# warlock-labs/sylow

Hardware: AMD Instinct MI355X
Metric: BN254 pairings/s (value) and BLS verifies/s (config.bls_verifies_per_s) at batch=2^20 per GPU (higher is better)
Workload: dtype i32/u32 limbs (9x29-bit carry-free core + 8x32-bit Montgomery, exact integer)

## Files before the change

sylow_amd/csrc/bn254_pair29.hpp:

```cpp
#pragma once
#include "bn254_f29.hpp"
#include "bn254_pair.hpp"

namespace bn254 {
namespace pl {

struct W2 { F29 c; };
BN_DEV const F29& f29_of(const W2& a) { return a.c; }
BN_DEV F29& f29_of(W2& a) { return a.c; }
struct W6 { W2 c0, c1, c2; };
struct W12 { W6 c0, c1; };

BN_DEV F29 xchg9(const F29& a) {
  F29 r;
#pragma unroll
  for (int i = 0; i < 9; ++i) r.v[i] = (i32)swap_u32((u32)a.v[i]);
  return r;
}
BN_DEV F29 sel9(bool odd, const F29& if_even, const F29& if_odd) {
  F29 r;
#pragma unroll
  for (int i = 0; i < 9; ++i) r.v[i] = odd ? if_odd.v[i] : if_even.v[i];
  return r;
}
BN_DEV F29 f29_reduce(const F29& a) {
  const F29* const x[1] = {&a};
  const i32 k[1] = {bn_keep(1)};
  return f29_reduce_terms(x, k);
}

#define BN_DPP_SWAP "row_half_mirror row_mask:0xf bank_mask:0xf"
#define BN_DPP_SWAP_C0 "row_half_mirror row_mask:0xf bank_mask:0x5"
#define BN_DPP_SELF_C0 "quad_perm:[0,1,2,3] row_mask:0xf bank_mask:0x5"
BN_DEV void w2_exchange(const F29& a, F29& b, F29& U, F29& W) {
  asm("s_nop 1\n\ts_mov_b32 vcc_lo, 0x0f0f0f0f\n\ts_mov_b32 vcc_hi, 0x0f0f0f0f\n\t"
      "v_cndmask_b32_dpp %0, %9, %9, vcc " BN_DPP_SWAP "\n\tv_cndmask_b32_dpp %1, %10, %10, vcc " BN_DPP_SWAP "\n\t"
      "v_cndmask_b32_dpp %2, %11, %11, vcc " BN_DPP_SWAP "\n\tv_cndmask_b32_dpp %3, %12, %12, vcc " BN_DPP_SWAP "\n\t"
      "v_cndmask_b32_dpp %4, %13, %13, vcc " BN_DPP_SWAP "\n\tv_cndmask_b32_dpp %5, %14, %14, vcc " BN_DPP_SWAP "\n\t"
      "v_cndmask_b32_dpp %6, %15, %15, vcc " BN_DPP_SWAP "\n\tv_cndmask_b32_dpp %7, %16, %16, vcc " BN_DPP_SWAP "\n\t"
// ... 14 lines not shown
      "v_mov_b32_dpp %0, %0 " BN_DPP_SWAP_C0 "\n\tv_mov_b32_dpp %1, %1 " BN_DPP_SWAP_C0 "\n\t"
      "v_mov_b32_dpp %2, %2 " BN_DPP_SWAP_C0 "\n\tv_mov_b32_dpp %3, %3 " BN_DPP_SWAP_C0 "\n\t"
      "v_mov_b32_dpp %4, %4 " BN_DPP_SWAP_C0 "\n\tv_mov_b32_dpp %5, %5 " BN_DPP_SWAP_C0 "\n\t"
      "v_mov_b32_dpp %6, %6 " BN_DPP_SWAP_C0 "\n\tv_mov_b32_dpp %7, %7 " BN_DPP_SWAP_C0 "\n\t"
      "v_mov_b32_dpp %8, %8 " BN_DPP_SWAP_C0 "\n\t"
      "v_sub_u32_dpp %0, %9, %0 " BN_DPP_SELF_C0 "\n\tv_sub_u32_dpp %1, %9, %1 " BN_DPP_SELF_C0 "\n\t"
      "v_sub_u32_dpp %2, %9, %2 " BN_DPP_SELF_C0 "\n\tv_sub_u32_dpp %3, %9, %3 " BN_DPP_SELF_C0 "\n\t"
      "v_sub_u32_dpp %4, %9, %4 " BN_DPP_SELF_C0 "\n\tv_sub_u32_dpp %5, %9, %5 " BN_DPP_SELF_C0 "\n\t"
      "v_sub_u32_dpp %6, %9, %6 " BN_DPP_SELF_C0 "\n\tv_sub_u32_dpp %7, %9, %7 " BN_DPP_SELF_C0 "\n\t"
      "v_sub_u32_dpp %8, %9, %8 " BN_DPP_SELF_C0
      : "+v"(b.v[0]), "+v"(b.v[1]), "+v"(b.v[2]), "+v"(b.v[3]), "+v"(b.v[4]), "+v"(b.v[5]), "+v"(b.v[6]), "+v"(b.v[7]), "+v"(b.v[8])
      : "v"(zero));
}
BN_NOINLINE F29 w2_mul_leaf(i32 a0, i32 a1, i32 a2, i32 a3, i32 a4, i32 a5, i32 a6, i32 a7, i32 a8,
                            i32 b0, i32 b1, i32 b2, i32 b3, i32 b4, i32 b5, i32 b6, i32 b7, i32 b8) {
  const F29 a{{a0, a1, a2, a3, a4, a5, a6, a7, a8}};
  F29 b{{b0, b1, b2, b3, b4, b5, b6, b7, b8}}, U, W;
  w2_exchange(a, b, U, W);
  return f29_dot2(a, U, W, b);
}
BN_NOINLINE F29 w2_mul_ilp_leaf(i32 a0, i32 a1, i32 a2, i32 a3, i32 a4, i32 a5, i32 a6, i32 a7, i32 a8,
                                i32 b0, i32 b1, i32 b2, i32 b3, i32 b4, i32 b5, i32 b6, i32 b7, i32 b8) {
  const F29 a{{a0, a1, a2, a3, a4, a5, a6, a7, a8}};
  F29 b{{b0, b1, b2, b3, b4, b5, b6, b7, b8}}, U, W;
  w2_exchange(a, b, U, W);
  return f29_dot2_ilp(a, U, W, b);
}
BN_NOINLINE F29 w2_sqr_leaf(i32 a0, i32 a1, i32 a2, i32 a3, i32 a4, i32 a5, i32 a6, i32 a7, i32 a8) {
  const F29 a{{a0, a1, a2, a3, a4, a5, a6, a7, a8}};
  const bool odd = lane_odd();
  const F29 o = xchg9(a);
  return f29_mul(sel9(odd, f29_add(a, o), o), sel9(odd, f29_sub(a, o), f29_dbl(a)));
}
BN_DEV W2 w2_mul(const W2& a, const W2& b) { return W2{w2_mul_leaf(W_ARGS(a.c), W_ARGS(b.c))}; }
BN_DEV W2 w2_mul_inl(const W2& a, const W2& bin) {
  F29 b = bin.c, U, W;
  w2_exchange(a.c, b, U, W);
  return W2{f29_dot2(a.c, U, W, b)};
}
BN_DEV W2 w2_mul_ilp(const W2& a, const W2& b) { return W2{w2_mul_ilp_leaf(W_ARGS(a.c), W_ARGS(b.c))}; }
BN_DEV W2 w2_sqr(const W2& a) { return W2{w2_sqr_leaf(W_ARGS(a.c))}; }
BN_DEV W2 w2_scale(const W2& a, const F29& k) { return W2{f29_mul_leaf(W_ARGS(a.c), W_ARGS(k))}; }

#ifndef BN_QUAD
#define BN_QUAD 0
#endif
#if BN_QUAD
template <class T> BN_DEV int quad_pair(T t) { return (int)((t & 3) ^ (((t >> 2) & 1) ? 3 : 0)); }
template <class T> BN_DEV T quad_index(T t) { return (T)(((t >> 3) << 1) | (T)(quad_pair(t) >> 1)); }
template <class T> BN_DEV int quad_sub(T t) { return quad_pair(t) & 1; }
BN_DEV bool quad_sub1() { return quad_sub(__lane_id()) != 0; }
BN_DEV F29 quad_xchg9(const F29& a) {
  F29 r;
#pragma unroll
  for (int i = 0; i < 9; ++i) r.v[i] = __builtin_amdgcn_mov_dpp(a.v[i], 0xB1, 0xF, 0xF, true);
  return r;
}
BN_DEV void quad_share(W2& r0, W2& r1, const F29& mine) {
  const bool s = quad_sub1();
  const F29 other = quad_xchg9(mine);
  r0 = W2{sel9(s, mine, other)};
  r1 = W2{sel9(s, other, mine)};
}
#endif
#if BN_QUAD
BN_DEV void w2_mul2(W2& r0, W2& r1, const W2& a0, const W2& b0, const W2& a1, const W2& b1) {
// ... 19 lines not shown
#define W2_SQR_MUL(r0, r1, a0, a1, b1) do { (r0) = w2_sqr(a0); (r1) = w2_mul(a1, b1); } while (0)
#define W2_SCALE2(r0, r1, a0, k0, a1, k1) do { (r0) = w2_scale(a0, k0); (r1) = w2_scale(a1, k1); } while (0)
#endif

BN_DEV W2 w2_add(const W2& a, const W2& b) { return W2{f29_add(a.c, b.c)}; }
BN_DEV W2 w2_sub(const W2& a, const W2& b) { return W2{f29_sub(a.c, b.c)}; }
BN_DEV W2 w2_neg(const W2& a) { return W2{f29_neg(a.c)}; }
BN_DEV W2 w2_norm(const W2& a) { return W2{f29_norm(a.c)}; }
BN_DEV W2 w2_reduce(const W2& a) { return W2{f29_reduce(a.c)}; }
BN_DEV W2 w2_lin2(const W2& a, int ka, const W2& b, int kb) { return W2{f29_lin2(a.c, ka, b.c, kb)}; }
BN_DEV W2 w2_xi_lin(const W2& x, int k, const W2& y, int m) {
  const F29 xo = xchg9(x.c);
  if (m == 0) {
    const F29* const t[2] = {&x.c, &xo};
    const i32 c[2] = {bn_keep(9 * k), bn_keep_v(lane_odd() ? k : -k)};
    return W2{f29_reduce_terms(t, c)};
  }
  const F29* const t[3] = {&x.c, &xo, &y.c};
  const i32 c[3] = {bn_keep(9 * k), bn_keep_v(lane_odd() ? k : -k), bn_keep(m)};
  return W2{f29_reduce_terms(t, c)};
}

BN_DEV W2 w2_from_s2(const S2& a) { return W2{f29_reduce(f29_from_fp(a.c))}; }
BN_DEV S2 w2_to_s2(const W2& a) { return S2{f29_to_fp(a.c)}; }
BN_DEV W2 w2_const(const uint32_t (&c)[2][8]) { return w2_from_s2(s2_const(c)); }
BN_DEV void w12_from_s12(W12& r, const S12& a) {
  r.c0.c0 = w2_from_s2(a.c0.c0); r.c0.c1 = w2_from_s2(a.c0.c1); r.c0.c2 = w2_from_s2(a.c0.c2);
  r.c1.c0 = w2_from_s2(a.c1.c0); r.c1.c1 = w2_from_s2(a.c1.c1); r.c1.c2 = w2_from_s2(a.c1.c2);
}
BN_DEV void w12_to_s12(S12& r, const W12& a) {
  r.c0.c0 = w2_to_s2(a.c0.c0); r.c0.c1 = w2_to_s2(a.c0.c1); r.c0.c2 = w2_to_s2(a.c0.c2);
  r.c1.c0 = w2_to_s2(a.c1.c0); r.c1.c1 = w2_to_s2(a.c1.c1); r.c1.c2 = w2_to_s2(a.c1.c2);
}

struct W6Raw { W2 v0, x0, y1, v2, y2; };
template <bool INL = false> BN_DEV W2 w2_mul_sel(const W2& a, const W2& b) { return INL ? w2_mul_inl(a, b) : w2_mul(a, b); }
template <bool INL = false>
BN_DEV W6Raw w6_mul_raw(const W6& a, const W6& b) {
  W2 v0, v1, v2, s0, s1, s2;
  W2_MUL2_SEL(INL, v0, v1, a.c0, b.c0, a.c1, b.c1);
  W2_MUL2_SEL(INL, v2, s0, a.c2, b.c2, w2_sub(a.c1, a.c2), w2_sub(b.c1, b.c2));
  W2_MUL2_SEL(INL, s1, s2, w2_sub(a.c0, a.c1), w2_sub(b.c0, b.c1), w2_sub(a.c0, a.c2), w2_sub(b.c0, b.c2));
  return W6Raw{v0, w2_sub(w2_add(v1, v2), s0), w2_sub(w2_add(v0, v1), s1), v2, w2_add(w2_sub(w2_add(v0, v2), s2), v1)};
}
template <bool INL = false>
BN_DEV W6 w6_mul(const W6& a, const W6& b) {
  const W6Raw m = w6_mul_raw<INL>(a, b);
  W6 r;
  r.c0 = w2_xi_lin(m.x0, 1, m.v0, 1);
  r.c1 = w2_xi_lin(m.v2, 1, m.y1, 1);
  r.c2 = w2_reduce(m.y2);
  return r;
}
BN_DEV W6 w6_add_norm(const W6& a, const W6& b) {
  return W6{w2_norm(w2_add(a.c0, b.c0)), w2_norm(w2_add(a.c1, b.c1)), w2_norm(w2_add(a.c2, b.c2))};
}
BN_DEV W6 w6_sub(const W6& a, const W6& b) { return W6{w2_sub(a.c0, b.c0), w2_sub(a.c1, b.c1), w2_sub(a.c2, b.c2)}; }

BN_DEV void w12_mul_c1(W12& r, const W6Raw& t2, const W6& t0, const W6& t1) {
  r.c1.c0 = w2_xi_lin(t2.x0, 1, w2_sub(w2_sub(t2.v0, t0.c0), t1.c0), 1);
  r.c1.c1 = w2_xi_lin(t2.v2, 1, w2_sub(w2_sub(t2.y1, t0.c1), t1.c1), 1);
  r.c1.c2 = w2_lin2(w2_sub(t2.y2, t0.c2), 1, t1.c2, -1);
}
BN_DEV W12 w12_mul(const W12& a, const W12& b) {
  const W6 t0 = w6_mul(a.c0, b.c0);
  const W6 t1 = w6_mul(a.c1, b.c1);
// ... 83 lines not shown
  W2 d0, d2, d4, p12, p54, p10, p34, p30, p52, q02, q24, q04;
  W2_MUL2(d0, d2, z0, x0, z2, x2);
  W2_MUL2(d4, p12, z4, x4, z1, x2);
  W2_MUL2(p54, p10, z5, x4, z1, x0);
  W2_MUL2(p34, p30, z3, x4, z3, x0);
  W2_MUL2(p52, q02, z5, x2, w2_sub(z0, z2), w2_sub(x0, x2));
  W2_MUL2(q24, q04, w2_sub(z2, z4), w2_sub(x2, x4), w2_sub(z0, z4), w2_sub(x0, x4));
  const W2 qs = w2_mul(w2_norm(w2_add(w2_add(z1, z3), z5)), w2_norm(w2_add(w2_add(x0, x2), x4)));
  W12 o;
  o.c0.c0 = w2_xi_lin(w2_add(p12, d4), 1, d0, 1);
  o.c0.c1 = w2_xi_lin(w2_add(p54, d2), 1, p10, 1);
  o.c0.c2 = w2_reduce(w2_add(w2_sub(w2_add(d0, d2), q02), p34));
  o.c1.c0 = w2_xi_lin(w2_sub(w2_add(d2, d4), q24), 1, p30, 1);
  o.c1.c1 = w2_xi_lin(p52, 1, w2_sub(w2_add(d0, d4), q04), 1);
  {
    const W2 sa = w2_add(w2_add(p12, p54), p10), sb = w2_add(w2_add(p34, p30), p52);
    const F29* const t[3] = {&qs.c, &sa.c, &sb.c};
    const i32 c[3] = {bn_keep(1), bn_keep(-1), bn_keep(-1)};
    o.c1.c2 = W2{f29_reduce_terms(t, c)};
  }
  return o;
}
BN_DEV W2 w2_xi_lin_v(const W2& x, const W2& y, i32 m) {
  const F29 xo = xchg9(x.c);
  const F29* const t[3] = {&x.c, &xo, &y.c};
  const i32 c[3] = {bn_keep(9), bn_keep_v(lane_odd() ? 1 : -1), bn_keep_v(m)};
  return W2{f29_reduce_terms(t, c)};
}
BN_DEV W2 w2_lin_v(const W2& x, const W2& y, i32 m) {
  const F29* const t[2] = {&x.c, &y.c};
  const i32 c[2] = {bn_keep(1), bn_keep_v(m)};
  return W2{f29_reduce_terms(t, c)};
}
BN_DEV W12 w12_sparse_mul_unit(const W12& f, i32 u, const W2& x4, const W2& x2) {
  const W2 z0 = f.c0.c0, z1 = f.c0.c1, z2 = f.c0.c2, z3 = f.c1.c0, z4 = f.c1.c1, z5 = f.c1.c2;
  W2 d2, d4, p12, p54, p34, p52, a02, a04, q24, q13;
  W2_MUL2(d2, d4, z2, x2, z4, x4);
  W2_MUL2(p12, p54, z1, x2, z5, x4);
  W2_MUL2(p34, p52, z3, x4, z5, x2);
  W2_MUL2(a02, a04, z0, x2, z0, x4);
  const W2 x24 = w2_sub(x2, x4);
  W2_MUL2(q24, q13, w2_sub(z2, z4), x24, w2_sub(z1, z3), x24);
  W12 o;
  o.c0.c0 = w2_xi_lin_v(w2_add(p12, d4), z0, u);
  o.c0.c1 = w2_xi_lin_v(w2_add(p54, d2), z1, u);
  o.c0.c2 = w2_lin_v(w2_add(a02, p34), z2, u);
  o.c1.c0 = w2_xi_lin_v(w2_sub(w2_add(d2, d4), q24), z3, u);
  {
    const F29 xo = xchg9(p52.c);
    const F29* const t[4] = {&p52.c, &xo, &a04.c, &z4.c};
    const i32 c[4] = {bn_keep(9), bn_keep_v(lane_odd() ? 1 : -1), bn_keep(1), bn_keep_v(u)};
    o.c1.c1 = W2{f29_reduce_terms(t, c)};
  }
  o.c1.c2 = w2_lin_v(w2_sub(w2_add(p12, p34), q13), z5, u);
  return o;
}
BN_DEV W2 w2_xi_norm(const W2& x, const W2& y) {
  const F29 xo = xchg9(x.c);
  const F29* const t[3] = {&x.c, &xo, &y.c};
  const i32 c[3] = {bn_keep(9), bn_keep_v(lane_odd() ? 1 : -1), bn_keep(1)};
  return W2{f29_norm_terms(t, c)};
}
BN_DEV W2 w2_xi_norm_sub(const W2& x, const W2& y) {
  const F29 xo = xchg9(x.c);
  const F29* const t[3] = {&x.c, &xo, &y.c};
  const i32 c[3] = {bn_keep(-9), bn_keep_v(lane_odd() ? -1 : 1), bn_keep(1)};
  return W2{f29_norm_terms(t, c)};
}
template <bool INL = false>
BN_DEV void w_fp4_square_fold(W2& out0, W2& m, const W2& a, const W2& b, const W2& z) {
  W2 w;
  W2_MUL2_SEL(INL, m, w, a, b, w2_sub(a, b), w2_xi_norm_sub(b, a));
  const F29 mo = xchg9(m.c);
  const F29* const t[4] = {&w.c, &m.c, &mo, &z.c};
  const i32 c[4] = {bn_keep(3), bn_keep(30), bn_keep_v(lane_odd() ? 3 : -3), bn_keep(-2)};
  out0 = W2{f29_reduce_terms(t, c)};
}
template <bool INL = false>
BN_DEV W12 w12_cyclotomic_sqr(const W12& f) {
  const W2 z0 = f.c0.c0, z4 = f.c0.c1, z3 = f.c0.c2, z2 = f.c1.c0, z1 = f.c1.c1, z5 = f.c1.c2;
  W2 m;
  W12 r;
  w_fp4_square_fold<INL>(r.c0.c0, m, z0, z1, z0);
  r.c1.c1 = w2_lin2(m, 6, z1, 2);
  w_fp4_square_fold<INL>(r.c0.c1, m, z2, z3, z4);
  r.c1.c2 = w2_lin2(m, 6, z5, 2);
  w_fp4_square_fold<INL>(r.c0.c2, m, z4, z5, z3);
  r.c1.c0 = w2_xi_lin(m, 6, z2, 2);
  return r;
}

BN_DEV F29 f29_halve(const F29& a) {
  i32 p[9]; f29_p(p);
  const i32 m = -(a.v[0] & 1);
  i32 lo[9];
  i32 c = 0;
#pragma unroll
  for (int i = 0; i < 8; ++i) {
    i32 t = a.v[i] + (p[i] & m) + c;
// ... 29 lines not shown
  W2 xy, xx, b, c, yz2, e;
  W2_MUL_SQR(xy, xx, r.x, r.y, r.x);
  const W2 a = w2_halve(xy);
  l2 = w2_norm(w2_triple(xx));
  W2_SQR2(b, c, r.y, r.z);
  if (ISO) {
    yz2 = w2_sqr(w2_norm(w2_add(r.y, r.z)));
    e = w2_mul_27m3u(c);
  } else {
    W2_SQR_MUL(yz2, e, w2_norm(w2_add(r.y, r.z)), w2_twist_b(), w2_norm(w2_triple(c)));
  }
  const W2 h = w2_norm(w2_sub(yz2, w2_add(b, c)));
  l1 = w2_neg(h);
  l0 = w2_xi_lin(w2_sub(e, b), 1, b, 0);
  const W2 f = w2_norm(w2_triple(e));
  W2_MUL2(r.z, r.x, b, h, a, w2_sub(b, f));
  const W2 g = w2_halve(w2_norm(w2_add(b, f)));
  W2 gg, ee;
  W2_SQR2(gg, ee, g, e);
  r.y = w2_lin2(gg, 1, ee, -3);
#else
  const W2 a = w2_halve(w2_mul(r.x, r.y));
  l2 = w2_norm(w2_triple(w2_sqr(r.x)));
  const W2 b = w2_sqr(r.y);
  const W2 c = w2_sqr(r.z);
  const W2 h = w2_norm(w2_sub(w2_sqr(w2_norm(w2_add(r.y, r.z))), w2_add(b, c)));
  const W2 e = ISO ? w2_mul_27m3u(c) : w2_mul(w2_twist_b(), w2_norm(w2_triple(c)));
  l1 = w2_neg(h);
  r.z = w2_mul(b, h);
  l0 = w2_xi_lin(w2_sub(e, b), 1, b, 0);
  const W2 f = w2_norm(w2_triple(e));
  r.x = w2_mul(a, w2_sub(b, f));
  const W2 g = w2_halve(w2_norm(w2_add(b, f)));
  r.y = w2_lin2(w2_sqr(g), 1, w2_sqr(e), -3);
#endif
}
BN_DEV void g2_addition_step29(G2W& r, const W2& bx, const W2& by, W2& l0, W2& l1, W2& l2) {
#if BN_QUAD
  W2 zbx, zby, ebx, dby;
  W2_MUL2(zbx, zby, r.z, bx, r.z, by);
  const W2 d = w2_sub(r.x, zbx);
  const W2 e = w2_sub(r.y, zby);
  W2_MUL2(ebx, dby, e, bx, d, by);
  l0 = w2_xi_lin(w2_sub(ebx, dby), 1, bx, 0);
  l1 = d;
  l2 = w2_neg(e);
  const W2 dn = w2_norm(d), en = w2_norm(e);
  W2 f, ee, h, i, zee, zh, dj, hy;
  W2_SQR2(f, ee, dn, en);
  W2_MUL2(h, i, dn, f, r.x, f);
  W2_MUL2(zee, zh, r.z, ee, r.z, h);
  const W2 j = w2_norm(w2_sub(w2_add(zee, h), w2_add(i, i)));
  W2_MUL2(dj, hy, dn, j, h, r.y);
  r.z = zh;
  r.x = dj;
  r.y = w2_norm(w2_sub(w2_mul(en, w2_sub(i, j)), hy));
#else
  const W2 d = w2_sub(r.x, w2_mul(r.z, bx));
  const W2 e = w2_sub(r.y, w2_mul(r.z, by));
  l0 = w2_xi_lin(w2_sub(w2_mul(e, bx), w2_mul(d, by)), 1, bx, 0);
  l1 = d;
  l2 = w2_neg(e);
  const W2 dn = w2_norm(d), en = w2_norm(e);
  const W2 f = w2_sqr(dn);
  const W2 h = w2_mul(dn, f);
  const W2 i = w2_mul(r.x, f);
  const W2 j = w2_norm(w2_sub(w2_add(w2_mul(r.z, w2_sqr(en)), h), w2_add(i, i)));
  r.z = w2_mul(r.z, h);
  r.x = w2_mul(dn, j);
  r.y = w2_norm(w2_sub(w2_mul(en, w2_sub(i, j)), w2_mul(h, r.y)));
#endif
}
BN_DEV W12 w12_line_product(const W2& a0, const W2& a4, const W2& a2, const W2& b0, const W2& b4, const W2& b2) {
  W2 d0, d2, d4, k02, k24, k04;
  W2_MUL2(d0, d2, a0, b0, a2, b2);
  W2_MUL2(d4, k02, a4, b4, w2_sub(a0, a2), w2_sub(b0, b2));
  W2_MUL2(k24, k04, w2_sub(a2, a4), w2_sub(b2, b4), w2_sub(a0, a4), w2_sub(b0, b4));
  W12 r;
  r.c0.c0 = w2_xi_lin(d4, 1, d0, 1);
  r.c0.c1 = w2_xi_lin(d2, 1, d2, 0);
  r.c0.c2 = w2_reduce(w2_sub(w2_add(d0, d2), k02));
  r.c1.c0 = w2_xi_lin(w2_sub(w2_add(d2, d4), k24), 1, d2, 0);
  r.c1.c1 = w2_reduce(w2_sub(w2_add(d0, d4), k04));
  r.c1.c2 = W2{F29{{0, 0, 0, 0, 0, 0, 0, 0, 0}}};
  return r;
}
constexpr int MILLER_LDS_WORDS = 36, MILLER_LDS_WORDS_PARK = 63;
BN_DEV void lds_put9(i32 (*lds)[256], int slot, const F29& a) {
#pragma unroll
  for (int i = 0; i < 9; ++i) lds[9 * slot + i][threadIdx.x] = a.v[i];
}
BN_DEV F29 lds_get9(i32 (*lds)[256], int slot) {
  F29 r;
#pragma unroll
  for (int i = 0; i < 9; ++i) r.v[i] = lds[9 * slot + i][threadIdx.x];
  return r;
}
#ifndef BN_MILLER_SQR_INL
#define BN_MILLER_SQR_INL false
#endif
template <bool PARK, bool ISO = false>
BN_NOINLINE void miller_loop29g(S12& fout, const Fp& pxs, const Fp& pys, const S2& qxs_in, const S2& qys_in) {
  __shared__ i32 lds[PARK ? MILLER_LDS_WORDS_PARK : MILLER_LDS_WORDS][256];
  S2 qxs = qxs_in, qys = qys_in;
  {
    const F29 px = f29_reduce(f29_from_fp(pxs)), py = f29_reduce(f29_from_fp(pys));
    lds_put9(lds, 0, ISO ? f29_mul(px, f29_iso_s2()) : px);
    lds_put9(lds, 1, ISO ? f29_mul(py, f29_iso_s3()) : py);
  }
  {
    W2 qx = w2_from_s2(qxs), qy = w2_from_s2(qys);
    if (ISO) {
      W2_SCALE2(qx, qy, qx, f29_iso_s2(), qy, f29_iso_s3());
      qxs = w2_to_s2(qx); qys = w2_to_s2(qy);
    }
    lds_put9(lds, 2, qx.c);
    lds_put9(lds, 3, qy.c);
  }
  auto PX = [&]() { return lds_get9(lds, 0); };
  auto PY = [&]() { return lds_get9(lds, 1); };
  auto QX = [&]() { return W2{lds_get9(lds, 2)}; };
  auto QY = [&](bool neg) { const W2 y{lds_get9(lds, 3)}; return neg ? w2_neg(y) : y; };
  auto park = [&](const G2W& r) { if (PARK) { lds_put9(lds, 4, r.x.c); lds_put9(lds, 5, r.y.c); lds_put9(lds, 6, r.z.c); } };
  auto unpark = [&](const G2W& r) { return PARK ? G2W{W2{lds_get9(lds, 4)}, W2{lds_get9(lds, 5)}, W2{lds_get9(lds, 6)}} : r; };
  W12 f;
  G2W r{QX(), QY(false), w2_from_s2(s2_one())};
  W2 l0, l1, l2;
  auto line_mul = [&](const W12& x) {
    W2 s1, s2;
    W2_SCALE2(s1, s2, l1, PY(), l2, PX());
    return w12_sparse_mul(x, l0, s1, s2);
  };
  const u64 nz = BN_ATE_NAF_NZ, ng = BN_ATE_NAF_NEG;
  static_assert((BN_ATE_NAF_NZ >> 63) & 1, "the first digit of 6x+2 after the leading one is non-zero");
  {
    g2_doubling_step29<ISO>(r, l0, l1, l2);
    const W2 d0 = l0;
    W2 d4, d2, e4, e2;
    W2_SCALE2(d4, d2, l1, PY(), l2, PX());
    g2_addition_step29(r, QX(), QY((ng >> 63) & 1), l0, l1, l2);
    park(r);
    W2_SCALE2(e4, e2, l1, PY(), l2, PX());
    f = w12_line_product(d0, d4, d2, l0, e4, e2);
  }
#pragma unroll 1
  for (int i = 1; i < 64; ++i) {
    r = unpark(r);
    g2_doubling_step29<ISO>(r, l0, l1, l2);
    park(r);
    f = w12_sqr<BN_MILLER_SQR_INL>(f);
    f = line_mul(f);
    if ((nz >> (63 - i)) & 1) {
      r = unpark(r);
      g2_addition_step29(r, QX(), QY((ng >> (63 - i)) & 1), l0, l1, l2);
      park(r);
      f = line_mul(f);
    }
  }
  r = unpark(r);
  S2 q1x, q1y, q2x, q2y;
  g2_psi_affine(q1x, q1y, qxs, qys);
  g2_psi_affine(q2x, q2y, q1x, q1y);
  q2y = s2_neg(q2y);
  g2_addition_step29(r, w2_from_s2(q1x), w2_from_s2(q1y), l0, l1, l2);
  f = line_mul(f);
  g2_addition_step29(r, w2_from_s2(q2x), w2_from_s2(q2y), l0, l1, l2);
  f = line_mul(f);
  w12_to_s12(fout, f);
}


BN_DEV void w12_pin(W12& x) {
  W2* const c[6] = {&x.c0.c0, &x.c0.c1, &x.c0.c2, &x.c1.c0, &x.c1.c1, &x.c1.c2};
#pragma unroll
  for (int j = 0; j < 6; ++j)
#pragma unroll
    for (int i = 0; i < 9; ++i) BN_CHAIN_NV(c[j]->c.v[i]);
}
BN_NOINLINE void w12_mul_nl(W12& r, const W12& a, const W12& b) {
  W12 x = a, y = b;
  w12_pin(x); w12_pin(y);
  r = w12_mul(x, y);
}
BN_NOINLINE void w12_cyclotomic_sqr_nl(W12& r, const W12& a) {
  W12 x = a;
  w12_pin(x);
  r = w12_cyclotomic_sqr(x);
}
template <int E> BN_NOINLINE void w12_frobenius_nl(W12& r, const W12& a) {
  W12 x = a;
  w12_pin(x);
  r = w12_frobenius<E>(x);
}
#ifndef BN_EXP_INL
#define BN_EXP_INL true
#endif
#define BN_X_C_NZ 0x0008144402208421ull
#define BN_X_C_NEG 0x0008004400000020ull
#define BN_X_C_17 0x0000100000008021ull
BN_NOINLINE void exp_by_neg_z29(W12& r, const W12& f) {
  W12 tab[2];
// ... 22 lines not shown
}
BN_DEV W2 w2_inv(const W2& a) {
  const F29 t = f29_mul_leaf(W_ARGS(a.c), W_ARGS(a.c));
  const F29 n = f29_norm(f29_add(t, xchg9(t)));
  const F29 i = f29_reduce(f29_from_fp(fp_inv(f29_to_fp(n))));
  const F29 r = f29_mul_leaf(W_ARGS(a.c), W_ARGS(i));
  return W2{sel9(lane_odd(), r, f29_norm(f29_neg(r)))};
}
BN_DEV W2 w2_mul_xi(const W2& a) { return w2_xi_lin(a, 1, a, 0); }
BN_DEV W6 w6_inv(const W6& a) {
  W2 s0, m12, s2, m01, s1, m02, u1, u2, o0, o1;
  W2_SQR_MUL(s0, m12, a.c0, a.c1, w2_mul_xi(a.c2));
  W2_SQR_MUL(s2, m01, a.c2, a.c0, a.c1);
  W2_SQR_MUL(s1, m02, a.c1, a.c0, a.c2);
  const W2 t0 = w2_sub(s0, m12);
  const W2 t1 = w2_sub(w2_mul_xi(s2), m01);
  const W2 t2 = w2_sub(s1, m02);
  W2_MUL2(u1, u2, a.c2, t1, a.c1, t2);
  const W2 d = w2_xi_lin(w2_add(u1, u2), 1, w2_mul(a.c0, t0), 1);
  const W2 di = w2_inv(d);
  W2_MUL2(o0, o1, di, t0, di, t1);
  return W6{o0, o1, w2_mul(di, t2)};
}
BN_NOINLINE void w12_inv_nl(W12& r, const W12& ain) {
  W12 a = ain;
  w12_pin(a);
  const W6 s0 = w6_mul(a.c0, a.c0), s1 = w6_mul(a.c1, a.c1);
  const W6 d{w2_norm(w2_sub(s0.c0, w2_mul_xi(s1.c2))), w2_norm(w2_sub(s0.c1, s1.c0)), w2_norm(w2_sub(s0.c2, s1.c1))};
  const W6 t = w6_inv(d);
  r.c0 = w6_mul(a.c0, t);
  const W6 m = w6_mul(a.c1, t);
  r.c1 = W6{w2_norm(w2_neg(m.c0)), w2_norm(w2_neg(m.c1)), w2_norm(w2_neg(m.c2))};
}
BN_NOINLINE void final_exponentiation29(S12& out, const S12& fin) {
  W12 in, t, a, b, d, e, g;
  {
    w12_from_s12(t, fin);
    w12_inv_nl(b, t);
    a = w12_conj(t);
    w12_mul_nl(d, a, b);
    w12_frobenius_nl<2>(a, d);
    w12_mul_nl(in, a, d);
  }
  exp_by_neg_z29(a, in);
  w12_cyclotomic_sqr_nl(b, a);
  w12_cyclotomic_sqr_nl(t, b);
  w12_mul_nl(d, t, b);
  exp_by_neg_z29(e, d);
  w12_cyclotomic_sqr_nl(t, e);
  exp_by_neg_z29(g, t);
  d = w12_conj(d);
  g = w12_conj(g);
  w12_mul_nl(t, g, e);
  w12_mul_nl(a, t, d);
  w12_mul_nl(d, a, b);
  w12_mul_nl(t, a, e);
  w12_mul_nl(e, in, t);
  w12_frobenius_nl<1>(t, d);
  w12_mul_nl(b, t, e);
  w12_frobenius_nl<2>(t, a);
  w12_mul_nl(e, t, b);
  t = w12_conj(in);
  w12_mul_nl(a, t, d);
  w12_frobenius_nl<3>(t, a);
  w12_mul_nl(g, t, e);
  w12_to_s12(out, g);
}


#ifdef BN_WIDE_LEAF_CALL
BN_DEV W2 w2_mul_w(const W2& a, const W2& b) { return w2_mul(a, b); }
#else
BN_DEV W2 w2_mul_w(const W2& a, const W2& b) { return w2_mul_inl(a, b); }
#endif
struct alignas(16) WideLds { i32 v[63][2][12]; };
typedef __attribute__((address_space(3))) WideLds* WideLdsPtr;
template <int EPW> BN_DEV int wide_j(int lane) { return (int)pair_index((u32)lane) & (32 / EPW - 1); }
typedef i32 __attribute__((ext_vector_type(4))) WideVec4;
typedef __attribute__((address_space(3))) WideVec4* WideVec4Ptr;
BN_DEV void wide_put(WideLdsPtr x, int slot, int odd, const W2& a) {
  const WideVec4Ptr p = (WideVec4Ptr)&x->v[slot][odd][0];
  p[0] = WideVec4{a.c.v[0], a.c.v[1], a.c.v[2], a.c.v[3]};
  p[1] = WideVec4{a.c.v[4], a.c.v[5], a.c.v[6], a.c.v[7]};
  x->v[slot][odd][8] = a.c.v[8];
}
BN_DEV W2 wide_get(WideLdsPtr x, int slot, int odd) {
  const WideVec4Ptr p = (WideVec4Ptr)&x->v[slot][odd][0];
  const WideVec4 lo = p[0], hi = p[1];
  W2 r;
  r.c.v[0] = lo.x; r.c.v[1] = lo.y; r.c.v[2] = lo.z; r.c.v[3] = lo.w;
  r.c.v[4] = hi.x; r.c.v[5] = hi.y; r.c.v[6] = hi.z; r.c.v[7] = hi.w;
  r.c.v[8] = x->v[slot][odd][8];
  return r;
}
BN_DEV W2 w2_pick(const W2& a, const W2& b, bool c) { return W2{sel9(c, a.c, b.c)}; }
BN_DEV W2 w2_real(const F29& k) { return W2{sel9(lane_odd(), k, F29{{0, 0, 0, 0, 0, 0, 0, 0, 0}})}; }
BN_DEV W2 w2_sel3(int k, const W2& a, const W2& b, const W2& c) { return w2_pick(w2_pick(a, b, k == 1), c, k == 2); }
template <int EPW = 1>
BN_DEV W12 w12_cyclotomic_sqr_wide(const W12& f, WideLdsPtr x) {
// ... 427 lines not shown
```

sylow_amd/csrc/plk_pairing.hip:

```cpp
#include "plk_common.hpp"

namespace plk {
__global__ void HEAVY_BOUNDS k_miller_loop(const u64* pxy, const u64* qxy, u64* fout, size_t n) {
  const size_t t = TID, i = pair_index(t);
  const int odd = pair_role(t);
  if (i >= n) return;
  const Fp px = load_fp(pxy, n, i, 0), py = load_fp(pxy, n, i, 4);
  const S2 qx = load_s2(qxy, n, i, 0, odd), qy = load_s2(qxy, n, i, 8, odd);
  S12 f;
  miller_loop29g<true>(f, px, py, qx, qy);
  store_s12(fout, n, i, odd, f);
}
__global__ void HEAVY_BOUNDS k_final_exp(const u64* fin, u64* gout, size_t n) {
  const size_t t = TID, i = pair_index(t);
  const int odd = pair_role(t);
  if (i >= n) return;
  S12 f, g;
  load_s12(f, fin, n, i, odd);
  final_exponentiation29(g, f);
  store_s12(gout, n, i, odd, g);
}
BN_DEV void pairing_body(const u64* pxy, const uint8_t* pinf, const u64* qxy, const uint8_t* qinf, u64* gout, size_t n, size_t m, const Stagger& st) {
  unsigned chunk;
  int role = stagger_role(st, chunk);
  const size_t t = (size_t)chunk * blockDim.x + threadIdx.x, i = pair_index(t);
  const int odd = pair_role(t);
  const size_t np = (size_t)st.count * (BLOCK / 2), ip = (size_t)(chunk - st.first) * (BLOCK / 2) + (i & (BLOCK / 2 - 1));
  if (role == 2 && !stagger_wait(st, chunk)) role = 0;
  if (role == 2) {
    S12 f, g;
    load_s12(f, st.park, np, ip, odd);
    final_exponentiation29(g, f);
    store_s12(gout, n, i, odd, g);
    return;
  }
  if (i >= m) return;
  const bool either_zero = (pinf && pinf[i]) || (qinf && qinf[i]);
  S12 g;
  if (either_zero) {
    g = s12_one();
    if (role == 1) store_s12(st.park, np, ip, odd, g);
  } else {
    const Fp px = load_fp(pxy, n, i, 0), py = load_fp(pxy, n, i, 4);
    const S2 qx = load_s2(qxy, n, i, 0, odd), qy = load_s2(qxy, n, i, 8, odd);
    S12 f;
    miller_loop29g<true, true>(f, px, py, qx, qy);
    if (role == 1) store_s12(st.park, np, ip, odd, f);
    else final_exponentiation29(g, f);
  }
  if (role == 1) { stagger_publish(st, chunk); return; }
  store_s12(gout, n, i, odd, g);
}
__global__ void HEAVY_BOUNDS k_pairing(const u64* pxy, const uint8_t* pinf, const u64* qxy, const uint8_t* qinf, u64* gout, size_t n, size_t m, Stagger st) {
  ClockProbe pb;
  probe_begin(pb, st.clk);
  pairing_body(pxy, pinf, qxy, qinf, gout, n, m, st);
  probe_end(pb, st.clk);
}

using namespace plkh;
__global__ void HEAVY_BOUNDS k_w12_op(int op, const u64* a, const u64* b, u64* out, size_t n) {
  const size_t t = TID, i = pair_index(t);
  const int odd = pair_role(t);
  if (i >= n) return;
  S12 sx, sy, sr;
  load_s12(sx, a, n, i, odd);
  if (op >= OPW_S_MUL && op <= OPW_S_CYCSQR) {
    if (b) load_s12(sy, b, n, i, odd);
    if (op == OPW_S_MUL) sr = s12_mul(sx, sy);
    else if (op == OPW_S_SQR) sr = s12_sqr(sx);
    else if (op == OPW_S_INV) sr = s12_inv(sx);
    else sr = cyclotomic_sqr(sx);
  } else {
    w12_hook_op(op - OPW_MUL, sr, sx, b, n, i, odd);
  }
  store_s12(out, n, i, odd, sr);
}
}

namespace plkh {
int32_t fp12_op(int32_t op, const uint64_t* a, const uint64_t* b, uint64_t* out, size_t n, void* stream) {
// ... 61 lines not shown
```

sylow_amd/csrc/plk_quad.hip:

```cpp
#define BN_QUAD 1
#include "plk_common.hpp"
#include "plk_verify_body.hpp"

namespace plk {
__global__ void HEAVY_BOUNDS k_pairing_quad(const u64* pxy, const uint8_t* pinf, const u64* qxy, const uint8_t* qinf, u64* gout, size_t n, size_t m, u64* clk) {
  const size_t t = TID, i = quad_index(t);
  const int odd = pair_role(t);
  if (i >= m) return;
  ClockProbe pb;
  probe_begin(pb, clk);
  __builtin_amdgcn_s_setprio(2);
  const bool either_zero = (pinf && pinf[i]) || (qinf && qinf[i]);
  S12 g;
  if (either_zero) {
    g = s12_one();
  } else {
    const Fp px = load_fp(pxy, n, i, 0), py = load_fp(pxy, n, i, 4);
    const S2 qx = load_s2(qxy, n, i, 0, odd), qy = load_s2(qxy, n, i, 8, odd);
    S12 f;
    miller_loop29g<true, true>(f, px, py, qx, qy);
    final_exponentiation29(g, f);
  }
  if (quad_sub(t) == 0) store_s12(gout, n, i, odd, g);
  probe_end(pb, clk);
}
__global__ void HEAVY_BOUNDS k_miller_loop_quad(const u64* pxy, const u64* qxy, u64* fout, size_t n) {
  const size_t t = TID, i = quad_index(t);
  const int odd = pair_role(t);
  if (i >= n) return;
  const Fp px = load_fp(pxy, n, i, 0), py = load_fp(pxy, n, i, 4);
  const S2 qx = load_s2(qxy, n, i, 0, odd), qy = load_s2(qxy, n, i, 8, odd);
  S12 f;
  miller_loop29g<true>(f, px, py, qx, qy);
  if (quad_sub(t) == 0) store_s12(fout, n, i, odd, f);
}
__global__ void HEAVY_BOUNDS k_final_exp_quad(const u64* fin, u64* gout, size_t n) {
  const size_t t = TID, i = quad_index(t);
  const int odd = pair_role(t);
  if (i >= n) return;
  S12 f, g;
  load_s12(f, fin, n, i, odd);
  final_exponentiation29(g, f);
  if (quad_sub(t) == 0) store_s12(gout, n, i, odd, g);
}
template <bool PK_TABLE>
__global__ void HEAVY_BOUNDS k_bls_verify_fused_quad(const u64* pkxy, const uint8_t* pkinf, const i32* pk_table, const u64* hneg, const uint8_t* hneg_inf,
                                                     const u64* sigxy, const uint8_t* siginf, const i32* gen_table, uint8_t* okout, size_t n, size_t m, u64* clk) {
  const Stagger none{0, 0, 0, 0, nullptr, nullptr, nullptr};
  __builtin_amdgcn_s_setprio(2);
  ClockProbe pb;
  probe_begin(pb, clk);
  bls_verify_fused_body<PK_TABLE>(pkxy, pkinf, pk_table, hneg, hneg_inf, sigxy, siginf, gen_table, okout, n, m, none);
// ... 48 lines not shown
```

sylow_amd/csrc/plk_verify.hip:

```cpp
#include "plk_common.hpp"
#include "plk_verify_body.hpp"

namespace plk {
BN_DEV bool hash_to_g1_pair(Fp& hx, Fp& hy, bool& hinf, const uint8_t* msg, size_t msg_len, const DstPrime& dp) {
  const bool odd = lane_odd();
  u64 em[12], half[6];
  expand_message_xmd96_words(em, msg, msg_len, dp);
#pragma unroll
  for (int k = 0; k < 6; ++k) half[k] = odd ? em[6 + k] : em[k];
  const Fp u = fp_from_be48_words(half);
  Fp x, y;
  u32 ok = svdw_map(x, y, u) ? 1u : 0u;
  ok &= swap_u32(ok);
  const Fp ox = xchg(x), oy = xchg(y);
  const G1P a{sel(odd, x, ox), sel(odd, y, oy), fp_one()}, b{sel(odd, ox, x), sel(odd, oy, y), fp_one()};
  const G1P h = g1_add(a, b);
  g1_to_affine(hx, hy, hinf, h);
  return ok != 0;
}

constexpr int LINES_BLOCK = 192;
__global__ void __launch_bounds__(LINES_BLOCK) k_g2_lines29(const u64* qxy, size_t n, size_t idx, i32* table) {
  __shared__ i32 raw[LINE_TABLE_LINES][3][2][9];
  const int odd = pair_role(threadIdx.x);
  if (pair_index(threadIdx.x) == 0) {
    S2 qxs = s2_g2gen_x(), qys = s2_g2gen_y();
    if (qxy) { qxs = load_s2(qxy, n, idx, 0, odd); qys = load_s2(qxy, n, idx, 8, odd); }
    const W2 qx = w2_from_s2(qxs), qy = w2_from_s2(qys), nqy = w2_from_s2(s2_neg(qys));
    G2W r{qx, qy, w2_from_s2(s2_one())};
    W2 l0, l1, l2;
    int at = 0;
    auto put = [&]() {
      const W2 c[3] = {l0, w2_reduce(l1), w2_reduce(l2)};
      for (int k = 0; k < 3; ++k) for (int j = 0; j < 9; ++j) raw[at][k][odd][j] = c[k].c.v[j];
      ++at;
    };
    const u64 nz = BN_ATE_NAF_NZ, ng = BN_ATE_NAF_NEG;
#pragma unroll 1
    for (int i = 0; i < 64; ++i) {
      g2_doubling_step29(r, l0, l1, l2); put();
      if ((nz >> (63 - i)) & 1) { g2_addition_step29(r, qx, ((ng >> (63 - i)) & 1) ? nqy : qy, l0, l1, l2); put(); }
    }
    S2 q1x, q1y, q2x, q2y;
    g2_psi_affine(q1x, q1y, qxs, qys);
    g2_psi_affine(q2x, q2y, q1x, q1y);
    g2_addition_step29(r, w2_from_s2(q1x), w2_from_s2(q1y), l0, l1, l2); put();
    g2_addition_step29(r, w2_from_s2(q2x), w2_from_s2(s2_neg(q2y)), l0, l1, l2); put();
  }
  __syncthreads();
  const int line = (int)(pair_index(threadIdx.x));
  if (line >= LINE_TABLE_LINES) return;
  auto get = [&](int k) {
    const i32* t = raw[line][k][odd];
    return W2{F29{{t[0], t[1], t[2], t[3], t[4], t[5], t[6], t[7], t[8]}}};
  };
  const W2 l0 = get(0), l1 = get(1), l2 = get(2);
  u32 nzero = 0;
  for (int j = 0; j < 9; ++j) nzero |= (u32)l0.c.v[j];
  nzero |= swap_u32(nzero);
  const bool unit = nzero != 0;
  const W2 inv = w2_inv(l0);
  const W2 c[2] = {unit ? w2_reduce(w2_mul(l1, inv)) : l1, unit ? w2_reduce(w2_mul(l2, inv)) : l2};
  for (int k = 0; k < 2; ++k) for (int j = 0; j < 9; ++j) table[((line * 2 + k) * 2 + odd) * 9 + j] = c[k].c.v[j];
  if (!odd) table[LINE_TABLE_LINES * 36 + line] = unit ? 1 : 0;
}
__global__ void HEAVY_BOUNDS k_bls_verify(const u64* pkxy, const uint8_t* pkinf, const uint8_t* msgs, const u64* off, DstPrime dp,
                                          const u64* sigxy, const uint8_t* siginf, const i32* gen_table, uint8_t* okout, size_t n) {
  __shared__ i32 tabA[LINE_TABLE_WORDS];
  stage_table(tabA, gen_table);
  __syncthreads();
  const size_t t = TID, i = pair_index(t);
  const int odd = pair_role(t);
  if (i >= n) return;
  Fp hx, hy; bool hinf;
  hash_to_g1_pair(hx, hy, hinf, msgs + off[i], (size_t)(off[i + 1] - off[i]), dp);
  S12 lhs, rhs;
  if (siginf && siginf[i]) {
    lhs = s12_one();
  } else {
    const F29 sx = f29_reduce(f29_from_fp(load_fp(sigxy, n, i, 0))), sy = f29_reduce(f29_from_fp(load_fp(sigxy, n, i, 4)));
// ... 222 lines not shown
```

sylow_amd/csrc/plk_verify_body.hpp:

```cpp
#pragma once
#include "plk_common.hpp"

namespace plk {
BN_DEV void stage_table(i32* lds, const i32* src) {
  for (int k = threadIdx.x; k < LINE_TABLE_WORDS; k += blockDim.x) lds[k] = src[k];
}
BN_DEV W2 table_w2(const i32* tab, int at, int c, int odd) {
  const i32* t = tab + ((at * 2 + c) * 2 + odd) * 9;
  return W2{F29{{t[0], t[1], t[2], t[3], t[4], t[5], t[6], t[7], t[8]}}};
}
BN_DEV i32 table_unit(const i32* tab, int at) { return tab[LINE_TABLE_LINES * 36 + at]; }

template <bool PK_TABLE>
BN_DEV void bls_verify_fused_body(const u64* pkxy, const uint8_t* pkinf, const i32* pk_table,
                                  const u64* hneg, const uint8_t* hneg_inf,
                                  const u64* sigxy, const uint8_t* siginf, const i32* gen_table, uint8_t* okout, size_t n, size_t m, const Stagger& st) {
  __shared__ i32 tabA[LINE_TABLE_WORDS];
  __shared__ i32 tabB[PK_TABLE ? LINE_TABLE_WORDS : 1];
  unsigned chunk;
  int role = stagger_role(st, chunk);
  const size_t t = (size_t)chunk * blockDim.x + threadIdx.x, i = elem_index(t);
  const int odd = pair_role(t);
  const size_t np = (size_t)st.count * ELEMS_PER_BLOCK, ip = (size_t)(chunk - st.first) * ELEMS_PER_BLOCK + (i & (ELEMS_PER_BLOCK - 1));
  if (role == 2 && !stagger_wait(st, chunk)) role = 0;
  if (role == 2) {
    S12 fs, g;
    load_s12(fs, st.park, np, ip, odd);
    final_exponentiation29(g, fs);
    const bool one = s12_is_one(g);
    if (!odd && elem_writer(t)) okout[i] = one ? 1 : 0;
    return;
  }
  stage_table(tabA, gen_table);
  if (PK_TABLE) stage_table(tabB, pk_table);
  __syncthreads();
  const bool active = i < m;
  const size_t ii = active ? i : 0;
  const Fp hxs = load_fp(hneg, n, ii, 0), hys = load_fp(hneg, n, ii, 4);
  const bool hinf = hneg_inf[ii] != 0;
  __shared__ i32 lds[PK_TABLE ? 36 : 54][256];
  const bool liveA = !(siginf && siginf[ii]);
  const bool liveB = !(hinf || (pkinf && pkinf[PK_TABLE ? 0 : ii]));
  const F29 f29_zero{{0, 0, 0, 0, 0, 0, 0, 0, 0}};
  lds_put9(lds, 0, liveA ? f29_reduce(f29_from_fp(load_fp(sigxy, n, ii, 0))) : f29_zero);
  lds_put9(lds, 1, liveA ? f29_reduce(f29_from_fp(load_fp(sigxy, n, ii, 4))) : f29_zero);
  constexpr bool ISO = !PK_TABLE;
  lds_put9(lds, 2, liveB ? (ISO ? f29_mul(f29_reduce(f29_from_fp(hxs)), f29_iso_s2()) : f29_reduce(f29_from_fp(hxs))) : f29_zero);
  lds_put9(lds, 3, liveB ? (ISO ? f29_mul(f29_reduce(f29_from_fp(hys)), f29_iso_s3()) : f29_reduce(f29_from_fp(hys))) : f29_zero);
  auto SX = [&]() { return lds_get9(lds, 0); };
  auto SY = [&]() { return lds_get9(lds, 1); };
  auto HX = [&]() { return lds_get9(lds, 2); };
  auto HY = [&]() { return lds_get9(lds, 3); };
  auto key_x = [&]() { return (PK_TABLE || !liveB) ? s2_g2gen_x() : load_s2(pkxy, n, ii, 0, odd); };
  auto key_y = [&]() { return (PK_TABLE || !liveB) ? s2_g2gen_y() : load_s2(pkxy, n, ii, 8, odd); };
  G2W r;
  {
    W2 qx = w2_from_s2(key_x()), qy = w2_from_s2(key_y());
    if (ISO) W2_SCALE2(qx, qy, qx, f29_iso_s2(), qy, f29_iso_s3());
    if (!PK_TABLE) { lds_put9(lds, 4, qx.c); lds_put9(lds, 5, qy.c); }
    r = G2W{qx, qy, w2_from_s2(s2_one())};
  }
// ... 17 lines not shown
  auto lineB = [&]() {
    if (PK_TABLE) {
      W2 b1, b2;
      W2_SCALE2(b1, b2, table_w2(tabB, idx, 0, odd), HY(), table_w2(tabB, idx, 1, odd), HX());
      f = w12_sparse_mul_unit(f, liveB ? table_unit(tabB, idx) : 1, b1, b2);
    } else {
      W2 s1, s2;
      W2_SCALE2(s1, s2, l1, HY(), l2, HX());
      f = w12_sparse_mul(f, l0, s1, s2);
    }
  };
  const u64 nz = BN_ATE_NAF_NZ, ng = BN_ATE_NAF_NEG;
#pragma unroll 1
  for (int it = 0; it < 64; ++it) {
    f = w12_sqr(f);
    lineA();
    if (!PK_TABLE) g2_doubling_step29<ISO>(r, l0, l1, l2);
    lineB();
    ++idx;
    if ((nz >> (63 - it)) & 1) {
      lineA();
      if (!PK_TABLE) g2_addition_step29(r, QX(), QY(((ng >> (63 - it)) & 1) != 0), l0, l1, l2);
      lineB();
      ++idx;
    }
  }
  S2 q1x, q1y, q2x, q2y;
  if (!PK_TABLE) { g2_psi_affine(q1x, q1y, w2_to_s2(QX()), w2_to_s2(QY(false))); g2_psi_affine(q2x, q2y, q1x, q1y); }
  lineA();
  if (!PK_TABLE) g2_addition_step29(r, w2_from_s2(q1x), w2_from_s2(q1y), l0, l1, l2);
  lineB();
  ++idx;
  lineA();
  if (!PK_TABLE) g2_addition_step29(r, w2_from_s2(q2x), w2_from_s2(s2_neg(q2y)), l0, l1, l2);
  lineB();
  S12 fs, g;
  w12_to_s12(fs, f);
  if (role == 1) {
    store_s12(st.park, np, ip, odd, fs);
    stagger_publish(st, chunk);
    return;
  }
  final_exponentiation29(g, fs);
  const bool one = s12_is_one(g);
  if (active && !odd && elem_writer(t)) okout[i] = one ? 1 : 0;
}
}
```

Baseline: 9.552 million.

## Trim redundant field work in sparse line mul, doubling, final addition and easy-part exponentiation

```diff
diff --git a/sylow_amd/csrc/bn254_pair29.hpp b/sylow_amd/csrc/bn254_pair29.hpp
--- a/sylow_amd/csrc/bn254_pair29.hpp
+++ b/sylow_amd/csrc/bn254_pair29.hpp
@@ -5,6 +5,9 @@
 namespace bn254 {
 namespace pl {
 
+#ifndef BN_TRIM
+#define BN_TRIM 15
+#endif
 struct W2 { F29 c; };
 BN_DEV const F29& f29_of(const W2& a) { return a.c; }
 BN_DEV F29& f29_of(W2& a) { return a.c; }
@@ -85,6 +88,17 @@
   const F29 o = xchg9(a);
   return f29_mul(sel9(odd, f29_add(a, o), o), sel9(odd, f29_sub(a, o), f29_dbl(a)));
 }
+BN_NOINLINE F29 w2_sqr2_sub3_leaf(i32 g0, i32 g1, i32 g2, i32 g3, i32 g4, i32 g5, i32 g6, i32 g7, i32 g8,
+                                  i32 e0, i32 e1, i32 e2, i32 e3, i32 e4, i32 e5, i32 e6, i32 e7, i32 e8) {
+  const F29 g{{g0, g1, g2, g3, g4, g5, g6, g7, g8}}, e{{e0, e1, e2, e3, e4, e5, e6, e7, e8}};
+  const bool odd = lane_odd();
+  const F29 go = xchg9(g), eo = xchg9(e);
+  const F29 eoe = f29_sub(eo, e);
+  const F29 a = f29_norm(sel9(odd, f29_add(g, go), go)), b = f29_norm(sel9(odd, f29_sub(g, go), f29_dbl(g)));
+  const F29 c = f29_norm(sel9(odd, f29_add(e, eo), f29_add(f29_dbl(eo), eo)));
+  const F29 d = f29_norm(sel9(odd, f29_add(f29_dbl(eoe), eoe), f29_neg(f29_dbl(e))));
+  return f29_dot2(a, b, c, d);
+}
 BN_DEV W2 w2_mul(const W2& a, const W2& b) { return W2{w2_mul_leaf(W_ARGS(a.c), W_ARGS(b.c))}; }
 BN_DEV W2 w2_mul_inl(const W2& a, const W2& bin) {
   F29 b = bin.c, U, W;
@@ -170,6 +184,11 @@
   r.c0.c0 = w2_to_s2(a.c0.c0); r.c0.c1 = w2_to_s2(a.c0.c1); r.c0.c2 = w2_to_s2(a.c0.c2);
   r.c1.c0 = w2_to_s2(a.c1.c0); r.c1.c1 = w2_to_s2(a.c1.c1); r.c1.c2 = w2_to_s2(a.c1.c2);
 }
+BN_DEV void w12_hand(S12& r, const W12& a) { w12_to_s12(r, a); }
+BN_DEV void w12_hand(W12& r, const S12& a) { w12_from_s12(r, a); }
+BN_DEV void w12_hand(W12& r, const W12& a) { r = a; }
+BN_DEV void w12_hand(S12& r, const S12& a) { r = a; }
+using F12H = std::conditional_t<(BN_TRIM & 16) != 0, W12, S12>;
 
 struct W6Raw { W2 v0, x0, y1, v2, y2; };
 template <bool INL = false> BN_DEV W2 w2_mul_sel(const W2& a, const W2& b) { return INL ? w2_mul_inl(a, b) : w2_mul(a, b); }
@@ -319,23 +338,36 @@
   const i32 c[2] = {bn_keep(1), bn_keep_v(m)};
   return W2{f29_reduce_terms(t, c)};
 }
+BN_DEV W2 w2_xi_norm_sub(const W2& x, const W2& y) {
+  const F29 xo = xchg9(x.c);
+  const F29* const t[3] = {&x.c, &xo, &y.c};
+  const i32 c[3] = {bn_keep(-9), bn_keep_v(lane_odd() ? -1 : 1), bn_keep(1)};
+  return W2{f29_norm_terms(t, c)};
+}
 BN_DEV W12 w12_sparse_mul_unit(const W12& f, i32 u, const W2& x4, const W2& x2) {
   const W2 z0 = f.c0.c0, z1 = f.c0.c1, z2 = f.c0.c2, z3 = f.c1.c0, z4 = f.c1.c1, z5 = f.c1.c2;
-  W2 d2, d4, p12, p54, p34, p52, a02, a04, q24, q13;
+  W2 d2, d4, p12, p54, p34, a02, q24, q13, xs, ys;
   W2_MUL2(d2, d4, z2, x2, z4, x4);
   W2_MUL2(p12, p54, z1, x2, z5, x4);
-  W2_MUL2(p34, p52, z3, x4, z5, x2);
-  W2_MUL2(a02, a04, z0, x2, z0, x4);
   const W2 x24 = w2_sub(x2, x4);
-  W2_MUL2(q24, q13, w2_sub(z2, z4), x24, w2_sub(z1, z3), x24);
+  if (BN_TRIM & 1) {
+    W2_MUL2(p34, a02, z3, x4, z0, x2);
+    W2_MUL2(q24, q13, w2_sub(z2, z4), x24, w2_sub(z1, z3), x24);
+    xs = p54;
+    ys = w2_sub(a02, w2_mul(w2_xi_norm_sub(z5, z0), x24));
+  } else {
+    W2_MUL2(p34, xs, z3, x4, z5, x2);
+    W2_MUL2(a02, ys, z0, x2, z0, x4);
+    W2_MUL2(q24, q13, w2_sub(z2, z4), x24, w2_sub(z1, z3), x24);
+  }
   W12 o;
   o.c0.c0 = w2_xi_lin_v(w2_add(p12, d4), z0, u);
   o.c0.c1 = w2_xi_lin_v(w2_add(p54, d2), z1, u);
   o.c0.c2 = w2_lin_v(w2_add(a02, p34), z2, u);
   o.c1.c0 = w2_xi_lin_v(w2_sub(w2_add(d2, d4), q24), z3, u);
   {
-    const F29 xo = xchg9(p52.c);
-    const F29* const t[4] = {&p52.c, &xo, &a04.c, &z4.c};
+    const F29 xo = xchg9(xs.c);
+    const F29* const t[4] = {&xs.c, &xo, &ys.c, &z4.c};
     const i32 c[4] = {bn_keep(9), bn_keep_v(lane_odd() ? 1 : -1), bn_keep(1), bn_keep_v(u)};
     o.c1.c1 = W2{f29_reduce_terms(t, c)};
   }
@@ -346,12 +378,6 @@
   const F29 xo = xchg9(x.c);
   const F29* const t[3] = {&x.c, &xo, &y.c};
   const i32 c[3] = {bn_keep(9), bn_keep_v(lane_odd() ? 1 : -1), bn_keep(1)};
-  return W2{f29_norm_terms(t, c)};
-}
-BN_DEV W2 w2_xi_norm_sub(const W2& x, const W2& y) {
-  const F29 xo = xchg9(x.c);
-  const F29* const t[3] = {&x.c, &xo, &y.c};
-  const i32 c[3] = {bn_keep(-9), bn_keep_v(lane_odd() ? -1 : 1), bn_keep(1)};
   return W2{f29_norm_terms(t, c)};
 }
 template <bool INL = false>
@@ -447,10 +473,13 @@
   const W2 f = w2_norm(w2_triple(e));
   r.x = w2_mul(a, w2_sub(b, f));
   const W2 g = w2_halve(w2_norm(w2_add(b, f)));
-  r.y = w2_lin2(w2_sqr(g), 1, w2_sqr(e), -3);
+  if (BN_TRIM & 8) r.y = W2{w2_sqr2_sub3_leaf(W_ARGS(g.c), W_ARGS(e.c))};
+  else r.y = w2_lin2(w2_sqr(g), 1, w2_sqr(e), -3);
 #endif
 }
+template <bool LINE_ONLY = false>
 BN_DEV void g2_addition_step29(G2W& r, const W2& bx, const W2& by, W2& l0, W2& l1, W2& l2) {
+  constexpr bool STOP = LINE_ONLY && (BN_TRIM & 2);
 #if BN_QUAD
   W2 zbx, zby, ebx, dby;
   W2_MUL2(zbx, zby, r.z, bx, r.z, by);
@@ -460,6 +489,7 @@
   l0 = w2_xi_lin(w2_sub(ebx, dby), 1, bx, 0);
   l1 = d;
   l2 = w2_neg(e);
+  if (STOP) return;
   const W2 dn = w2_norm(d), en = w2_norm(e);
   W2 f, ee, h, i, zee, zh, dj, hy;
   W2_SQR2(f, ee, dn, en);
@@ -476,6 +506,7 @@
   l0 = w2_xi_lin(w2_sub(w2_mul(e, bx), w2_mul(d, by)), 1, bx, 0);
   l1 = d;
   l2 = w2_neg(e);
+  if (STOP) return;
   const W2 dn = w2_norm(d), en = w2_norm(e);
   const W2 f = w2_sqr(dn);
   const W2 h = w2_mul(dn, f);
@@ -514,8 +545,8 @@
 #ifndef BN_MILLER_SQR_INL
 #define BN_MILLER_SQR_INL false
 #endif
-template <bool PARK, bool ISO = false>
-BN_NOINLINE void miller_loop29g(S12& fout, const Fp& pxs, const Fp& pys, const S2& qxs_in, const S2& qys_in) {
+template <bool PARK, bool ISO = false, class F12>
+BN_NOINLINE void miller_loop29g(F12& fout, const Fp& pxs, const Fp& pys, const S2& qxs_in, const S2& qys_in) {
   __shared__ i32 lds[PARK ? MILLER_LDS_WORDS_PARK : MILLER_LDS_WORDS][256];
   S2 qxs = qxs_in, qys = qys_in;
   {
@@ -579,9 +610,9 @@
   q2y = s2_neg(q2y);
   g2_addition_step29(r, w2_from_s2(q1x), w2_from_s2(q1y), l0, l1, l2);
   f = line_mul(f);
-  g2_addition_step29(r, w2_from_s2(q2x), w2_from_s2(q2y), l0, l1, l2);
+  g2_addition_step29<true>(r, w2_from_s2(q2x), w2_from_s2(q2y), l0, l1, l2);
   f = line_mul(f);
-  w12_to_s12(fout, f);
+  w12_hand(fout, f);
 }
 
 
@@ -670,13 +701,30 @@
   const W6 m = w6_mul(a.c1, t);
   r.c1 = W6{w2_norm(w2_neg(m.c0)), w2_norm(w2_neg(m.c1)), w2_norm(w2_neg(m.c2))};
 }
-BN_NOINLINE void final_exponentiation29(S12& out, const S12& fin) {
+BN_NOINLINE void w12_conj_over_nl(W12& r, const W12& ain) {
+  W12 a = ain;
+  w12_pin(a);
+  const W6 m = w6_mul(a.c0, a.c1);
+  const W6 m2{w2_norm(w2_neg(w2_add(m.c0, m.c0))), w2_norm(w2_neg(w2_add(m.c1, m.c1))), w2_norm(w2_neg(w2_add(m.c2, m.c2)))};
+  const W6 s0 = w6_mul(a.c0, a.c0), s1 = w6_mul(a.c1, a.c1);
+  const W2 vs = w2_mul_xi(s1.c2);
+  const W6 d{w2_norm(w2_sub(s0.c0, vs)), w2_norm(w2_sub(s0.c1, s1.c0)), w2_norm(w2_sub(s0.c2, s1.c1))};
+  const W6 t = w6_inv(d);
+  r.c0 = w6_mul(W6{w2_norm(w2_add(s0.c0, vs)), w2_norm(w2_add(s0.c1, s1.c0)), w2_norm(w2_add(s0.c2, s1.c1))}, t);
+  r.c1 = w6_mul(m2, t);
+}
+template <class F12>
+BN_NOINLINE void final_exponentiation29(S12& out, const F12& fin) {
   W12 in, t, a, b, d, e, g;
   {
-    w12_from_s12(t, fin);
-    w12_inv_nl(b, t);
-    a = w12_conj(t);
-    w12_mul_nl(d, a, b);
+    w12_hand(t, fin);
+    if (BN_TRIM & 4) {
+      w12_conj_over_nl(d, t);
+    } else {
+      w12_inv_nl(b, t);
+      a = w12_conj(t);
+      w12_mul_nl(d, a, b);
+    }
     w12_frobenius_nl<2>(a, d);
     w12_mul_nl(in, a, d);
   }
@@ -703,6 +751,25 @@
   w12_frobenius_nl<3>(t, a);
   w12_mul_nl(g, t, e);
   w12_to_s12(out, g);
+}
+BN_DEV void final_exponentiation29_acc(S12& out, const W12& f) {
+  if (BN_TRIM & 16) {
+    const W12 fh = f;
+    final_exponentiation29(out, fh);
+  } else {
+    S12 fs;
+    w12_to_s12(fs, f);
+    final_exponentiation29(out, fs);
+  }
+}
+BN_DEV void final_exponentiation29_parked(S12& out, const S12& fs) {
+  if (BN_TRIM & 16) {
+    W12 f;
+    w12_from_s12(f, fs);
+    final_exponentiation29(out, f);
+  } else {
+    final_exponentiation29(out, fs);
+  }
 }
 
 
diff --git a/sylow_amd/csrc/plk_pairing.hip b/sylow_amd/csrc/plk_pairing.hip
--- a/sylow_amd/csrc/plk_pairing.hip
+++ b/sylow_amd/csrc/plk_pairing.hip
@@ -28,9 +28,9 @@
   const size_t np = (size_t)st.count * (BLOCK / 2), ip = (size_t)(chunk - st.first) * (BLOCK / 2) + (i & (BLOCK / 2 - 1));
   if (role == 2 && !stagger_wait(st, chunk)) role = 0;
   if (role == 2) {
-    S12 f, g;
-    load_s12(f, st.park, np, ip, odd);
-    final_exponentiation29(g, f);
+    S12 fs, g;
+    load_s12(fs, st.park, np, ip, odd);
+    final_exponentiation29_parked(g, fs);
     store_s12(gout, n, i, odd, g);
     return;
   }
@@ -43,10 +43,15 @@
   } else {
     const Fp px = load_fp(pxy, n, i, 0), py = load_fp(pxy, n, i, 4);
     const S2 qx = load_s2(qxy, n, i, 0, odd), qy = load_s2(qxy, n, i, 8, odd);
-    S12 f;
+    F12H f;
     miller_loop29g<true, true>(f, px, py, qx, qy);
-    if (role == 1) store_s12(st.park, np, ip, odd, f);
-    else final_exponentiation29(g, f);
+    if (role == 1) {
+      S12 fs;
+      w12_hand(fs, f);
+      store_s12(st.park, np, ip, odd, fs);
+    } else {
+      final_exponentiation29(g, f);
+    }
   }
   if (role == 1) { stagger_publish(st, chunk); return; }
   store_s12(gout, n, i, odd, g);
diff --git a/sylow_amd/csrc/plk_quad.hip b/sylow_amd/csrc/plk_quad.hip
--- a/sylow_amd/csrc/plk_quad.hip
+++ b/sylow_amd/csrc/plk_quad.hip
@@ -17,7 +17,7 @@
   } else {
     const Fp px = load_fp(pxy, n, i, 0), py = load_fp(pxy, n, i, 4);
     const S2 qx = load_s2(qxy, n, i, 0, odd), qy = load_s2(qxy, n, i, 8, odd);
-    S12 f;
+    F12H f;
     miller_loop29g<true, true>(f, px, py, qx, qy);
     final_exponentiation29(g, f);
   }
diff --git a/sylow_amd/csrc/plk_verify.hip b/sylow_amd/csrc/plk_verify.hip
--- a/sylow_amd/csrc/plk_verify.hip
+++ b/sylow_amd/csrc/plk_verify.hip
@@ -45,7 +45,7 @@
     g2_psi_affine(q1x, q1y, qxs, qys);
     g2_psi_affine(q2x, q2y, q1x, q1y);
     g2_addition_step29(r, w2_from_s2(q1x), w2_from_s2(q1y), l0, l1, l2); put();
-    g2_addition_step29(r, w2_from_s2(q2x), w2_from_s2(s2_neg(q2y)), l0, l1, l2); put();
+    g2_addition_step29<true>(r, w2_from_s2(q2x), w2_from_s2(s2_neg(q2y)), l0, l1, l2); put();
   }
   __syncthreads();
   const int line = (int)(pair_index(threadIdx.x));
diff --git a/sylow_amd/csrc/plk_verify_body.hpp b/sylow_amd/csrc/plk_verify_body.hpp
--- a/sylow_amd/csrc/plk_verify_body.hpp
+++ b/sylow_amd/csrc/plk_verify_body.hpp
@@ -26,7 +26,7 @@
   if (role == 2) {
     S12 fs, g;
     load_s12(fs, st.park, np, ip, odd);
-    final_exponentiation29(g, fs);
+    final_exponentiation29_parked(g, fs);
     const bool one = s12_is_one(g);
     if (!odd && elem_writer(t)) okout[i] = one ? 1 : 0;
     return;
@@ -110,16 +110,17 @@
   lineB();
   ++idx;
   lineA();
-  if (!PK_TABLE) g2_addition_step29(r, w2_from_s2(q2x), w2_from_s2(s2_neg(q2y)), l0, l1, l2);
+  if (!PK_TABLE) g2_addition_step29<true>(r, w2_from_s2(q2x), w2_from_s2(s2_neg(q2y)), l0, l1, l2);
   lineB();
-  S12 fs, g;
-  w12_to_s12(fs, f);
+  S12 g;
   if (role == 1) {
+    S12 fs;
+    w12_to_s12(fs, f);
     store_s12(st.park, np, ip, odd, fs);
     stagger_publish(st, chunk);
     return;
   }
-  final_exponentiation29(g, fs);
+  final_exponentiation29_acc(g, f);
   const bool one = s12_is_one(g);
   if (active && !odd && elem_writer(t)) okout[i] = one ? 1 : 0;
 }
```

Result: no change. 9.616 million, median of 6 (+0.7%).
